# NjuHaoZhang/AMMCNet_AAAI2021

Hardware: AMD Instinct MI355X
Metric: frames/sec, 256x256x4 dual-stream clips (twostream forward, inference) (higher is better)
Workload: dtype f32-equivalent: (hi,lo) f16 split, 3 fp16 MFMAs per product (v_mfma_f32_32x32x16_f16 in the 4-wave k-half-major kernels, 16x16x32 in the 8-wave / fused-decoder kernels), f32 accumulate; 1 GPU; Ped2 full dual-stream + 2000-slot memory module, batch=16, inference (BASELINE.json configs[1]); batch_per_gpu=16, frame=256x256, n_embed=2000, embed_dim=64, k=2, parallelism=replicas x1 (no collective)

## Files before the change

### ammcnet_aaai2021_amd/csrc/conv_first_s16.hip

```cpp
#include "ammc_common.h"
#include <hip/hip_fp16.h>

namespace ammc_s16 {

typedef _Float16 f16x8v __attribute__((ext_vector_type(8)));

constexpr float F_LO_SCALE = 2048.f;
constexpr float F_LO_INV = 1.f / 2048.f;
constexpr int F_TH = 8, F_TW = 32, F_HW = F_TW + 2, F_HP = (F_TH + 2) * F_HW;
constexpr int F_NQ = 20;
constexpr int F_WFLOATS = F_NQ * 2 * 64 * 4;
constexpr int F_PFLOATS = F_HP * 16;

struct FirstArgs {
  const float* x;
  const float* w;
  const float* scale;
  const float* shift;
  float* y;
  int32_t* overflow_flag;
  int64_t y_bs, y_rs, y_ps;
  int64_t x_bs;
  int batch, c, h, w_, act, tiles_x, tiles_y;
};

template <int CT>
__device__ __forceinline__ int first_load_patch(const FirstArgs& a, int t, int tid, float (&v)[2][16]) {
  int sp = t;
  const int tx = sp % a.tiles_x;
  sp /= a.tiles_x;
  const int ty = sp % a.tiles_y;
  const int b = sp / a.tiles_y;
  const int plane = a.h * a.w_;
  const int nc = CT ? CT : a.c;
  const float* xb = a.x + (int64_t)b * a.x_bs;
  int inb = 0;
#pragma unroll
  for (int rnd = 0; rnd < 2; ++rnd) {
    const int P = rnd * 256 + tid;
    const int hy = P / F_HW, hx = P - hy * F_HW;
    const int yy = ty * F_TH - 1 + hy, xx = tx * F_TW - 1 + hx;
    const bool in = P < F_HP && yy >= 0 && yy < a.h && xx >= 0 && xx < a.w_;
    const int pix = in ? yy * a.w_ + xx : 0;
    inb |= in ? (1 << rnd) : 0;
#pragma unroll
    for (int c = 0; c < 16; ++c) {
      if (CT && c >= CT) {
        v[rnd][c] = 0.f;
      } else {
        const int cc = CT ? c : (c < nc ? c : nc - 1);
        v[rnd][c] = xb[cc * plane + pix];
      }
    }
  }
  return inb;
}

__device__ __forceinline__ void first_store_patch(float* Ps, int tid, const float (&v)[2][16], int inb, int nc) {
#pragma unroll
  for (int rnd = 0; rnd < 2; ++rnd) {
    const int P = rnd * 256 + tid;
    if (P < F_HP) {
      f16x8v hi[2], lo[2];
      const bool in = (inb >> rnd) & 1;
#pragma unroll
      for (int g = 0; g < 2; ++g) {
        float val[8];
#pragma unroll
        for (int c = 0; c < 8; ++c) val[c] = (in && 8 * g + c < nc) ? v[rnd][8 * g + c] : 0.f;
        ammc_u4 h, l;
        ammc_s16_split8(val, h, l);
        hi[g] = __builtin_bit_cast(f16x8v, h);
        lo[g] = __builtin_bit_cast(f16x8v, l);
      }
      const int sw = (P >> 2) & 1;
      float* pp = Ps + P * 16;
      *reinterpret_cast<f16x8v*>(pp + ((0 ^ sw) << 2)) = hi[0];
      *reinterpret_cast<f16x8v*>(pp + ((1 ^ sw) << 2)) = lo[0];
      *reinterpret_cast<f16x8v*>(pp + ((2 ^ sw) << 2)) = hi[1];
      *reinterpret_cast<f16x8v*>(pp + ((3 ^ sw) << 2)) = lo[1];
    }
  }
}

template <int CT>
__global__ __launch_bounds__(256, CT ? 2 : 1) void conv_first_s16_kernel(FirstArgs a) {
  extern __shared__ __attribute__((aligned(16))) float smem[];
  float* Ws = smem;
  float* Ps = smem + F_WFLOATS;

  const int tid = threadIdx.x, lane = tid & 63, wave = tid >> 6;
  const int l15 = lane & 15, g4 = lane >> 4;
  const int total = a.batch * a.tiles_y * a.tiles_x;

#pragma unroll
  for (int j = 0; j < F_WFLOATS / 4 / 256; ++j)
    __builtin_amdgcn_global_load_lds(a.w + (j * 256 + tid) * 4, Ws + (j * 256 + wave * 64) * 4, 16, 0, 0);

  float* Ss = Ps + F_PFLOATS;
  if (tid < 128) {
    const int c = tid & 63;
    Ss[tid] = tid < 64 ? (a.scale ? a.scale[c] : 1.f) : (a.shift ? a.shift[c] : 0.f);
  }

  float v[2][16];
  int t = blockIdx.x;
  const int nc = CT ? CT : a.c;
  int inb = first_load_patch<CT>(a, t, tid, v);
  first_store_patch(Ps, tid, v, inb, nc);
  asm volatile("s_waitcnt vmcnt(0) lgkmcnt(0)" ::: "memory");
  __builtin_amdgcn_s_barrier();
  asm volatile("" ::: "memory");

  float vmax = 0.f;
  for (; t < total; t += gridDim.x) {
  const int tn = t + gridDim.x;
  if (tn < total) inb = first_load_patch<CT>(a, tn, tid, v);
  int sp = t;
  const int tx = sp % a.tiles_x;
  sp /= a.tiles_x;
  const int ty = sp % a.tiles_y;
  const int b = sp / a.tiles_y;
  const int y0 = ty * F_TH, x0 = tx * F_TW;

  f32x4 acc[4][4];
#pragma unroll
  for (int i = 0; i < 4; ++i)
#pragma unroll
    for (int j = 0; j < 4; ++j) acc[i][j] = f32x4{0.f, 0.f, 0.f, 0.f};

#pragma unroll
  for (int kb = 0; kb < 5; ++kb) {
    const int q = 4 * kb + g4;
    const int tap = (q >> 1) < 9 ? (q >> 1) : 8;
    const int off = (tap / 3) * F_HW + (tap % 3);
    const int cg = q & 1;
    f16x8v ah[4], ax[4], al2[4];
#pragma unroll
    for (int pt = 0; pt < 4; ++pt) {
      const int P = (2 * wave + (pt >> 1)) * F_HW + 16 * (pt & 1) + l15 + off;
      const int sw = (P >> 2) & 1;
      const float* pp = Ps + P * 16;
      ah[pt] = *reinterpret_cast<const f16x8v*>(pp + (((2 * cg) ^ sw) << 2));
      const f16x8v al = *reinterpret_cast<const f16x8v*>(pp + (((2 * cg + 1) ^ sw) << 2));
      ax[pt] = ah[pt] * (_Float16)F_LO_INV;
      al2[pt] = al * (_Float16)F_LO_INV;
    }
    const float* wq = Ws + q * (2 * 64 * 4);
#pragma unroll
    for (int f0 = 0; f0 < 4; f0 += 2) {
      f16x8v bh[2], bl[2];
#pragma unroll
      for (int j = 0; j < 2; ++j) {
        bh[j] = *reinterpret_cast<const f16x8v*>(wq + ((f0 + j) * 16 + l15) * 4);
        bl[j] = *reinterpret_cast<const f16x8v*>(wq + 64 * 4 + ((f0 + j) * 16 + l15) * 4);
      }
#pragma unroll
      for (int pt = 0; pt < 4; ++pt)
#pragma unroll
        for (int j = 0; j < 2; ++j) acc[pt][f0 + j] = __builtin_amdgcn_mfma_f32_16x16x32_f16(bh[j], ah[pt], acc[pt][f0 + j], 0, 0, 0);
#pragma unroll
      for (int pt = 0; pt < 4; ++pt)
#pragma unroll
        for (int j = 0; j < 2; ++j) acc[pt][f0 + j] = __builtin_amdgcn_mfma_f32_16x16x32_f16(bl[j], ax[pt], acc[pt][f0 + j], 0, 0, 0);
#pragma unroll
      for (int pt = 0; pt < 4; ++pt)
#pragma unroll
        for (int j = 0; j < 2; ++j) acc[pt][f0 + j] = __builtin_amdgcn_mfma_f32_16x16x32_f16(bh[j], al2[pt], acc[pt][f0 + j], 0, 0, 0);
    }
  }

  if (tn < total) {
    asm volatile("" ::: "memory");
    __builtin_amdgcn_s_barrier();
    asm volatile("" ::: "memory");
    first_store_patch(Ps, tid, v, inb, nc);
    asm volatile("s_waitcnt lgkmcnt(0)" ::: "memory");
    __builtin_amdgcn_s_barrier();
    asm volatile("" ::: "memory");
  }

#pragma unroll
  for (int u = 0; u < 2; ++u) {
    const int c0 = 32 * u + 8 * g4;
    float sc[8], sh[8];
    {
      const f32x4 s0 = *reinterpret_cast<const f32x4*>(Ss + c0), s1 = *reinterpret_cast<const f32x4*>(Ss + c0 + 4);
      const f32x4 h0 = *reinterpret_cast<const f32x4*>(Ss + 64 + c0), h1 = *reinterpret_cast<const f32x4*>(Ss + 64 + c0 + 4);
#pragma unroll
      for (int k = 0; k < 4; ++k) sc[k] = s0[k], sc[4 + k] = s1[k], sh[k] = h0[k], sh[4 + k] = h1[k];
    }
#pragma unroll
    for (int pt = 0; pt < 4; ++pt) {
      const int y = y0 + 2 * wave + (pt >> 1), x = x0 + 16 * (pt & 1) + l15;
      float tv[8];
#pragma unroll
      for (int k = 0; k < 8; ++k) {
        tv[k] = acc[pt][2 * u + (k >> 2)][k & 3] * sc[k] + sh[k];
        if (a.act == AMMC_ACT_RELU) tv[k] = fmaxf(tv[k], 0.f);
      }
#pragma unroll
      for (int k = 0; k < 8; k += 2) vmax = fmaxf(vmax, fmaxf(fabsf(tv[k]), fabsf(tv[k + 1])));
      ammc_u4 hi, lo;
      ammc_s16_split8(tv, hi, lo);
      ammc_u4* yp = reinterpret_cast<ammc_u4*>(a.y + ((int64_t)b * a.y_bs + (int64_t)y * a.y_rs + (int64_t)x * a.y_ps) + c0);
      yp[0] = hi;
      yp[1] = lo;
    }
  }
  }
  if (a.overflow_flag && !(vmax <= 65504.f)) atomicOr(a.overflow_flag, 1);
}

__global__ __launch_bounds__(256) void pack_first_conv_kernel(const float* __restrict__ w, int cin, float* __restrict__ out) {
  const int gid = blockIdx.x * 256 + threadIdx.x;
  if (gid >= F_NQ * 64) return;
  const int q = gid / 64, pos = gid % 64;
  const int t = pos >> 4, r = pos & 15;
  const int f = 32 * (t >> 1) + 8 * (r >> 2) + 4 * (t & 1) + (r & 3);
  const int tap = q >> 1, cg = q & 1;
  f16x8v hi, lo;
#pragma unroll
  for (int i = 0; i < 8; ++i) {
    const int c = 8 * cg + i;
    const float v = (tap < 9 && c < cin) ? w[((int64_t)f * cin + c) * 9 + tap] : 0.f;
    const _Float16 hv = (_Float16)v;
    hi[i] = hv;
    lo[i] = (_Float16)((v - (float)hv) * F_LO_SCALE);
  }
  *reinterpret_cast<f16x8v*>(out + ((q * 2 + 0) * 64 + pos) * 4) = hi;
  *reinterpret_cast<f16x8v*>(out + ((q * 2 + 1) * 64 + pos) * 4) = lo;
}

}
using namespace ammc_s16;

extern "C" int ammc_first_conv_image_floats(void) { return F_WFLOATS; }

extern "C" int ammc_pack_first_conv_f32(const float* w_oihw, int32_t cout, int32_t cin, float* out, void* stream) {
  if (!w_oihw || !out) return AMMC_EINVAL;
  if (cout != 64 || cin <= 0 || cin > 16) return AMMC_EUNSUP;
  hipLaunchKernelGGL(pack_first_conv_kernel, dim3((F_NQ * 64 + 255) / 256), dim3(256), 0, (hipStream_t)stream, w_oihw, cin, out);
  return ammc_launch_status();
}

extern "C" int ammc_conv_first_s16(const float* x_nchw, int32_t batch, int32_t c, int32_t h, int32_t w,
                                   const float* w_image, const float* scale, const float* shift, int32_t act,
                                   float* y, int64_t y_bs, int64_t y_rs, int64_t y_ps, int32_t* overflow_flag, void* stream) {
  return ammc_conv_first_s16_bs(x_nchw, (int64_t)c * h * w, batch, c, h, w, w_image, scale, shift, act, y, y_bs, y_rs, y_ps,
                                overflow_flag, stream);
}

extern "C" int ammc_conv_first_s16_bs(const float* x_nchw, int64_t x_bs, int32_t batch, int32_t c, int32_t h, int32_t w,
                                      const float* w_image, const float* scale, const float* shift, int32_t act,
                                      float* y, int64_t y_bs, int64_t y_rs, int64_t y_ps, int32_t* overflow_flag,
                                      void* stream) {
  if (!x_nchw || !w_image || !y || batch <= 0 || c <= 0 || h <= 0 || w <= 0 || x_bs < 0) return AMMC_EINVAL;
  if (c > 16 || w % F_TW || h % F_TH) return AMMC_EUNSUP;
  if (act != AMMC_ACT_NONE && act != AMMC_ACT_RELU) return AMMC_EUNSUP;
  if (((uintptr_t)w_image & 15) || ((uintptr_t)y & 31) || ((y_bs | y_rs | y_ps) & 7)) return AMMC_EINVAL;
  if ((int64_t)batch * y_bs >= (1LL << 31)) return AMMC_EUNSUP;
  constexpr size_t lds = (size_t)(F_WFLOATS + F_PFLOATS + 128) * sizeof(float);
  static_assert(lds <= 80 * 1024, "two workgroups per CU");
  FirstArgs a;
  a.x = x_nchw, a.w = w_image, a.scale = scale, a.shift = shift, a.y = y, a.overflow_flag = overflow_flag;
  a.y_bs = y_bs, a.y_rs = y_rs, a.y_ps = y_ps, a.x_bs = x_bs;
  a.batch = batch, a.c = c, a.h = h, a.w_ = w, a.act = act;
  a.tiles_x = w / F_TW, a.tiles_y = h / F_TH;
  if ((int64_t)c * h * w >= (1LL << 31)) return AMMC_EUNSUP;
  const int total = batch * a.tiles_y * a.tiles_x;
  const dim3 grid(total < 512 ? total : 512);
#define FIRST_LAUNCH(CT)                                                                                              \
  {                                                                                                                   \
    hipError_t e = hipFuncSetAttribute(reinterpret_cast<const void*>(conv_first_s16_kernel<CT>),                     \
                                       hipFuncAttributeMaxDynamicSharedMemorySize, (int)lds);                         \
    if (e != hipSuccess) return (int)e;                                                                               \
    hipLaunchKernelGGL(conv_first_s16_kernel<CT>, grid, dim3(256), lds, (hipStream_t)stream, a);                     \
  }
  if (c == 12) FIRST_LAUNCH(12) else if (c == 6) FIRST_LAUNCH(6) else FIRST_LAUNCH(0)
#undef FIRST_LAUNCH
  return ammc_launch_status();
}
```

Before: 2475 frames/s.

## Add narrow 6-channel layout for first conv with one tap per k-slot

For 6-channel inputs the first conv now packs each tap's 8 channels into a single k-slot instead of two 8-channel groups, cutting k-blocks from 5 to 3 and halving the patch LDS footprint. The smaller LDS lets the kernel target three workgroups per CU with a larger grid, and the k-loop is not unrolled to limit register use. Weight packing changes to match, with a new swizzle for the narrower patch rows. Risks include lower ILP from the rolled loop and bank conflicts under the new swizzle.

```diff
diff --git a/ammcnet_aaai2021_amd/csrc/conv_first_s16.hip b/ammcnet_aaai2021_amd/csrc/conv_first_s16.hip
--- a/ammcnet_aaai2021_amd/csrc/conv_first_s16.hip
+++ b/ammcnet_aaai2021_amd/csrc/conv_first_s16.hip
@@ -7,10 +7,25 @@
 
 constexpr float F_LO_SCALE = 2048.f;
 constexpr float F_LO_INV = 1.f / 2048.f;
+#ifndef F_NARROW_OCC
+#define F_NARROW_OCC 3
+#endif
 constexpr int F_TH = 8, F_TW = 32, F_HW = F_TW + 2, F_HP = (F_TH + 2) * F_HW;
 constexpr int F_NQ = 20;
 constexpr int F_WFLOATS = F_NQ * 2 * 64 * 4;
-constexpr int F_PFLOATS = F_HP * 16;
+
+template <int CT>
+struct FirstLayout {
+  static constexpr bool NARROW = CT == 6;
+  static constexpr int NQ = NARROW ? 12 : F_NQ;
+  static constexpr int NKB = NQ / 4;
+  static constexpr int SP = NARROW ? 2 : 4;
+  static constexpr int NV = NARROW ? 8 : 16;
+  static constexpr int WFLOATS = NQ * 2 * 64 * 4;
+  static constexpr int PFLOATS = F_HP * 4 * SP;
+  static constexpr int OCC = NARROW ? F_NARROW_OCC : (CT ? 2 : 1);
+  static constexpr size_t LDS = (size_t)(WFLOATS + PFLOATS + 128) * sizeof(float);
+};
 
 struct FirstArgs {
   const float* x;
@@ -25,7 +40,7 @@
 };
 
 template <int CT>
-__device__ __forceinline__ int first_load_patch(const FirstArgs& a, int t, int tid, float (&v)[2][16]) {
+__device__ __forceinline__ int first_load_patch(const FirstArgs& a, int t, int tid, float (&v)[2][FirstLayout<CT>::NV]) {
   int sp = t;
   const int tx = sp % a.tiles_x;
   sp /= a.tiles_x;
@@ -44,7 +59,7 @@
     const int pix = in ? yy * a.w_ + xx : 0;
     inb |= in ? (1 << rnd) : 0;
 #pragma unroll
-    for (int c = 0; c < 16; ++c) {
+    for (int c = 0; c < FirstLayout<CT>::NV; ++c) {
       if (CT && c >= CT) {
         v[rnd][c] = 0.f;
       } else {
@@ -56,15 +71,17 @@
   return inb;
 }
 
-__device__ __forceinline__ void first_store_patch(float* Ps, int tid, const float (&v)[2][16], int inb, int nc) {
+template <int CT>
+__device__ __forceinline__ void first_store_patch(float* Ps, int tid, const float (&v)[2][FirstLayout<CT>::NV], int inb, int nc) {
+  using L = FirstLayout<CT>;
 #pragma unroll
   for (int rnd = 0; rnd < 2; ++rnd) {
     const int P = rnd * 256 + tid;
     if (P < F_HP) {
-      f16x8v hi[2], lo[2];
+      f16x8v hi[L::NV / 8], lo[L::NV / 8];
       const bool in = (inb >> rnd) & 1;
 #pragma unroll
-      for (int g = 0; g < 2; ++g) {
+      for (int g = 0; g < L::NV / 8; ++g) {
         float val[8];
 #pragma unroll
         for (int c = 0; c < 8; ++c) val[c] = (in && 8 * g + c < nc) ? v[rnd][8 * g + c] : 0.f;
@@ -73,41 +90,49 @@
         hi[g] = __builtin_bit_cast(f16x8v, h);
         lo[g] = __builtin_bit_cast(f16x8v, l);
       }
-      const int sw = (P >> 2) & 1;
-      float* pp = Ps + P * 16;
-      *reinterpret_cast<f16x8v*>(pp + ((0 ^ sw) << 2)) = hi[0];
-      *reinterpret_cast<f16x8v*>(pp + ((1 ^ sw) << 2)) = lo[0];
-      *reinterpret_cast<f16x8v*>(pp + ((2 ^ sw) << 2)) = hi[1];
-      *reinterpret_cast<f16x8v*>(pp + ((3 ^ sw) << 2)) = lo[1];
+      if constexpr (L::NARROW) {
+        const int sw = ((P >> 3) ^ (P >> 2)) & 1;
+        float* pp = Ps + P * 8;
+        *reinterpret_cast<f16x8v*>(pp + ((0 ^ sw) << 2)) = hi[0];
+        *reinterpret_cast<f16x8v*>(pp + ((1 ^ sw) << 2)) = lo[0];
+      } else {
+        const int sw = (P >> 2) & 1;
+        float* pp = Ps + P * 16;
+        *reinterpret_cast<f16x8v*>(pp + ((0 ^ sw) << 2)) = hi[0];
+        *reinterpret_cast<f16x8v*>(pp + ((1 ^ sw) << 2)) = lo[0];
+        *reinterpret_cast<f16x8v*>(pp + ((2 ^ sw) << 2)) = hi[1];
+        *reinterpret_cast<f16x8v*>(pp + ((3 ^ sw) << 2)) = lo[1];
+      }
     }
   }
 }
 
 template <int CT>
-__global__ __launch_bounds__(256, CT ? 2 : 1) void conv_first_s16_kernel(FirstArgs a) {
+__global__ __launch_bounds__(256, FirstLayout<CT>::OCC) void conv_first_s16_kernel(FirstArgs a) {
+  using L = FirstLayout<CT>;
   extern __shared__ __attribute__((aligned(16))) float smem[];
   float* Ws = smem;
-  float* Ps = smem + F_WFLOATS;
+  float* Ps = smem + L::WFLOATS;
 
   const int tid = threadIdx.x, lane = tid & 63, wave = tid >> 6;
   const int l15 = lane & 15, g4 = lane >> 4;
   const int total = a.batch * a.tiles_y * a.tiles_x;
 
 #pragma unroll
-  for (int j = 0; j < F_WFLOATS / 4 / 256; ++j)
+  for (int j = 0; j < L::WFLOATS / 4 / 256; ++j)
     __builtin_amdgcn_global_load_lds(a.w + (j * 256 + tid) * 4, Ws + (j * 256 + wave * 64) * 4, 16, 0, 0);
 
-  float* Ss = Ps + F_PFLOATS;
+  float* Ss = Ps + L::PFLOATS;
   if (tid < 128) {
     const int c = tid & 63;
     Ss[tid] = tid < 64 ? (a.scale ? a.scale[c] : 1.f) : (a.shift ? a.shift[c] : 0.f);
   }
 
-  float v[2][16];
+  float v[2][L::NV];
   int t = blockIdx.x;
   const int nc = CT ? CT : a.c;
   int inb = first_load_patch<CT>(a, t, tid, v);
-  first_store_patch(Ps, tid, v, inb, nc);
+  first_store_patch<CT>(Ps, tid, v, inb, nc);
   asm volatile("s_waitcnt vmcnt(0) lgkmcnt(0)" ::: "memory");
   __builtin_amdgcn_s_barrier();
   asm volatile("" ::: "memory");
@@ -129,18 +154,19 @@
 #pragma unroll
     for (int j = 0; j < 4; ++j) acc[i][j] = f32x4{0.f, 0.f, 0.f, 0.f};
 
-#pragma unroll
-  for (int kb = 0; kb < 5; ++kb) {
+  auto kblock = [&](const int kb) __attribute__((always_inline)) {
     const int q = 4 * kb + g4;
-    const int tap = (q >> 1) < 9 ? (q >> 1) : 8;
-    const int off = (tap / 3) * F_HW + (tap % 3);
-    const int cg = q & 1;
+    const int qt = L::NARROW ? q : (q >> 1);
+    const int tap = qt < 9 ? qt : 8;
+    const int trow = (tap * 11) >> 5;
+    const int off = trow * F_HW + (tap - 3 * trow);
+    const int cg = L::NARROW ? 0 : (q & 1);
     f16x8v ah[4], ax[4], al2[4];
 #pragma unroll
     for (int pt = 0; pt < 4; ++pt) {
       const int P = (2 * wave + (pt >> 1)) * F_HW + 16 * (pt & 1) + l15 + off;
-      const int sw = (P >> 2) & 1;
-      const float* pp = Ps + P * 16;
+      const int sw = L::NARROW ? ((P >> 3) ^ (P >> 2)) & 1 : (P >> 2) & 1;
+      const float* pp = Ps + P * (4 * L::SP);
       ah[pt] = *reinterpret_cast<const f16x8v*>(pp + (((2 * cg) ^ sw) << 2));
       const f16x8v al = *reinterpret_cast<const f16x8v*>(pp + (((2 * cg + 1) ^ sw) << 2));
       ax[pt] = ah[pt] * (_Float16)F_LO_INV;
@@ -168,13 +194,20 @@
 #pragma unroll
         for (int j = 0; j < 2; ++j) acc[pt][f0 + j] = __builtin_amdgcn_mfma_f32_16x16x32_f16(bh[j], al2[pt], acc[pt][f0 + j], 0, 0, 0);
     }
+  };
+  if constexpr (L::NARROW) {
+#pragma unroll 1
+    for (int kb = 0; kb < L::NKB; ++kb) kblock(kb);
+  } else {
+#pragma unroll
+    for (int kb = 0; kb < L::NKB; ++kb) kblock(kb);
   }
 
   if (tn < total) {
     asm volatile("" ::: "memory");
     __builtin_amdgcn_s_barrier();
     asm volatile("" ::: "memory");
-    first_store_patch(Ps, tid, v, inb, nc);
+    first_store_patch<CT>(Ps, tid, v, inb, nc);
     asm volatile("s_waitcnt lgkmcnt(0)" ::: "memory");
     __builtin_amdgcn_s_barrier();
     asm volatile("" ::: "memory");
@@ -214,11 +247,12 @@
 
 __global__ __launch_bounds__(256) void pack_first_conv_kernel(const float* __restrict__ w, int cin, float* __restrict__ out) {
   const int gid = blockIdx.x * 256 + threadIdx.x;
-  if (gid >= F_NQ * 64) return;
+  const bool narrow = cin == 6;
+  if (gid >= (narrow ? FirstLayout<6>::NQ : F_NQ) * 64) return;
   const int q = gid / 64, pos = gid % 64;
   const int t = pos >> 4, r = pos & 15;
   const int f = 32 * (t >> 1) + 8 * (r >> 2) + 4 * (t & 1) + (r & 3);
-  const int tap = q >> 1, cg = q & 1;
+  const int tap = narrow ? q : q >> 1, cg = narrow ? 0 : q & 1;
   f16x8v hi, lo;
 #pragma unroll
   for (int i = 0; i < 8; ++i) {
@@ -260,8 +294,8 @@
   if (act != AMMC_ACT_NONE && act != AMMC_ACT_RELU) return AMMC_EUNSUP;
   if (((uintptr_t)w_image & 15) || ((uintptr_t)y & 31) || ((y_bs | y_rs | y_ps) & 7)) return AMMC_EINVAL;
   if ((int64_t)batch * y_bs >= (1LL << 31)) return AMMC_EUNSUP;
-  constexpr size_t lds = (size_t)(F_WFLOATS + F_PFLOATS + 128) * sizeof(float);
-  static_assert(lds <= 80 * 1024, "two workgroups per CU");
+  static_assert(FirstLayout<12>::LDS <= 80 * 1024 && FirstLayout<0>::LDS <= 80 * 1024, "two workgroups per CU");
+  static_assert(FirstLayout<6>::LDS * FirstLayout<6>::OCC <= 160 * 1024, "FirstLayout<6>::OCC workgroups per CU");
   FirstArgs a;
   a.x = x_nchw, a.w = w_image, a.scale = scale, a.shift = shift, a.y = y, a.overflow_flag = overflow_flag;
   a.y_bs = y_bs, a.y_rs = y_rs, a.y_ps = y_ps, a.x_bs = x_bs;
@@ -269,9 +303,11 @@
   a.tiles_x = w / F_TW, a.tiles_y = h / F_TH;
   if ((int64_t)c * h * w >= (1LL << 31)) return AMMC_EUNSUP;
   const int total = batch * a.tiles_y * a.tiles_x;
-  const dim3 grid(total < 512 ? total : 512);
 #define FIRST_LAUNCH(CT)                                                                                              \
   {                                                                                                                   \
+    constexpr size_t lds = FirstLayout<CT>::LDS;                                                                      \
+    constexpr int full = 256 * (FirstLayout<CT>::OCC > 2 ? FirstLayout<CT>::OCC : 2);                                 \
+    const dim3 grid(total < full ? total : full);                                                                     \
     hipError_t e = hipFuncSetAttribute(reinterpret_cast<const void*>(conv_first_s16_kernel<CT>),                     \
                                        hipFuncAttributeMaxDynamicSharedMemorySize, (int)lds);                         \
     if (e != hipSuccess) return (int)e;                                                                               \
```

New measurement: 2304 frames/s. 0.931x the previous value.
